# ruivieira/ccfd-demo-summit

Hardware: AMD Instinct MI355X
Metric: transactions/sec (whole node) + p50 scoring latency at 1/2/4/8 MI355X (higher is better)
Workload: dtype bf16

## Files before the change

ccfd_demo_summit_amd/engine/stream_engine.py:

```python
from __future__ import annotations

import ctypes as C
import threading
import time
from dataclasses import dataclass, field
from typing import Dict, List, Optional

import numpy as np
import torch

from ..ops._lib import (BATCH_TRACE_DTYPE, BIN_FORMATS, ENGINE_FLAG_FULL, FLAGGED_DTYPE, SCORED_DTYPE, MODEL_IDS,
                        N_COUNTER_SLOTS, ROW_FORMATS, EngineConfig, EngineStats, Flagged, check, last_error, lib)
from ..ops._lib import (CNT_SHADOW_ABSDIFF_E6, CNT_SHADOW_BOTH, CNT_SHADOW_FRAUD, CNT_SHADOW_PROBA_E6,
                        CNT_SHADOW_ROWS)
from ..ops.kernels import ROW_BYTES, DeviceModel, check_shadow_pair

N_FEATURES = 30
WIRE_ROW_F32 = 16
G32_ROW_F32 = 8
G20_ROW_F32 = 5
INPUT_MODES = {"dma": 0, "zerocopy": 1}
OUTPUT_MODES = {"zerocopy": 0, "dma": 1}


# ... 615 lines not shown
        out = np.zeros(getattr(self, "_trace_cap", 0), BATCH_TRACE_DTYPE)
        if out.size == 0:
            return out
        n = lib().ccfd_engine_trace_read(C.c_void_p(self.h), out.ctypes.data, out.size)
        if n < 0:
            raise RuntimeError(f"ccfd_engine_trace_read failed: {last_error()}")
        return out[:n]

    def progress(self) -> Dict[str, int]:
        v = np.zeros(5, np.int64)
        if getattr(self, "h", None):
            lib().ccfd_engine_progress(C.c_void_p(self.h), v.ctypes.data)
        return {"submitted": int(v[0]), "completed": int(v[1]), "persist_posted": int(v[2]),
                "persist_resident": int(v[3]), "in_flight": int(v[4])}

    def emergency_stop(self, timeout_ms: int = 5000) -> int:
        if not getattr(self, "h", None):
            return 0
        return int(lib().ccfd_engine_emergency_stop(C.c_void_p(self.h), int(timeout_ms)))

    def cursor(self, partition: int) -> int:
        return int(lib().ccfd_engine_cursor(C.c_void_p(self.h), int(partition)))
```

ccfd_demo_summit_amd/ops/_lib.py:

```python
from __future__ import annotations

import ctypes as C
import os
import threading
from pathlib import Path

import torch

_NATIVE = Path(__file__).resolve().parents[1] / "_native"
_SAN = os.environ.get("CCFD_SANITIZE", "")
LIB_PATH = _NATIVE / (f"libccfd_hip_{_SAN.replace(',', '_')}.so" if _SAN else "libccfd_hip.so")
if os.environ.get("CCFD_LIB_PATH"):
    LIB_PATH = Path(os.environ["CCFD_LIB_PATH"]).resolve()

MODEL_LR, MODEL_MLP, MODEL_GBDT, MODEL_FOREST = 0, 1, 2, 3
MODEL_IDS = {"lr": MODEL_LR, "mlp": MODEL_MLP, "gbdt": MODEL_GBDT, "forest": MODEL_FOREST}
N_COUNTER_SLOTS = 64
ENGINE_FLAG_FULL = 1
CNT_WIRE_STALE = 4
CNT_SHADOW_ROWS, CNT_SHADOW_FRAUD, CNT_SHADOW_BOTH, CNT_SHADOW_PROBA_E6, CNT_SHADOW_ABSDIFF_E6 = 40, 41, 42, 43, 44
ARG_WIRE_W64, ARG_WIRE_G32, ARG_WIRE_G20 = 2, 4, 8
ROW_FORMATS = {"f32": 0, "w64": 1, "g32": 2, "g20": 3}
BIN_FORMATS = ("g32", "g20")

# ... 115 lines not shown
        L.ccfd_engine_drain_scored.argtypes = [C.c_void_p, C.c_void_p, C.c_int64]
        L.ccfd_engine_drain_scored.restype = C.c_int64
        L.ccfd_engine_scored_dropped.argtypes = [C.c_void_p]
        L.ccfd_engine_scored_dropped.restype = C.c_int64
        L.ccfd_engine_serve_start.argtypes = [C.c_void_p, C.c_int64, C.c_int64]
        L.ccfd_engine_serve_stop.argtypes = [C.c_void_p]
        L.ccfd_engine_serve_hold.argtypes = [C.c_void_p, C.c_int]
        L.ccfd_engine_serve_stats.argtypes = [C.c_void_p, C.POINTER(EngineStats), C.POINTER(C.c_int64)]
        L.ccfd_engine_serve_collect.argtypes = [C.c_void_p, C.POINTER(EngineStats), C.c_void_p, C.c_int64,
                                                C.POINTER(C.c_int64), C.c_void_p, C.c_int64, C.POINTER(C.c_int64)]
        L.ccfd_engine_cursor.argtypes = [C.c_void_p, C.c_int]
        L.ccfd_engine_cursor.restype = C.c_int64
        L.ccfd_engine_reset_stats.argtypes = [C.c_void_p]
        L.ccfd_engine_progress.argtypes = [C.c_void_p, C.c_void_p]
        L.ccfd_engine_emergency_stop.argtypes = [C.c_void_p, C.c_int]
        L.ccfd_engine_trace_enable.argtypes = [C.c_void_p, C.c_int32]
        L.ccfd_engine_trace_read.argtypes = [C.c_void_p, C.c_void_p, C.c_int32]
        L.ccfd_engine_set_ring.argtypes = [C.c_void_p, C.c_int, C.c_void_p, C.c_void_p, C.c_void_p, C.c_int64]
        L.ccfd_engine_ring_acquire.argtypes = [C.c_void_p, C.c_int, C.c_int64, C.POINTER(C.c_int64)]
        L.ccfd_engine_ring_acquire.restype = C.c_int64
        L.ccfd_engine_ring_commit.argtypes = [C.c_void_p, C.c_int, C.c_int64]
        L.ccfd_engine_ring_commit_at.argtypes = [C.c_void_p, C.c_int, C.c_int64, C.c_int64]
        L.ccfd_engine_run.argtypes = [C.c_void_p, C.c_int64, C.c_int64, C.POINTER(EngineStats)]
        L.ccfd_crc32c.argtypes = [C.c_char_p, C.c_size_t, C.c_uint32]
        L.ccfd_crc32c.restype = C.c_uint32
        L.ccfd_parse_json_batch.argtypes = [C.c_void_p, C.c_void_p, C.c_int64, C.c_void_p, C.c_void_p,
                                            C.c_void_p]
        L.ccfd_parse_json_batch.restype = C.c_int64
        L.ccfd_parse_json_batch_w64.argtypes = [C.c_void_p, C.c_void_p, C.c_int64, C.c_void_p, C.c_void_p,
                                                C.c_void_p]
# ... 33 lines not shown
```

csrc/engine/engine.cpp:

```cpp
#include <hip/hip_runtime_api.h>

#include <algorithm>
#include <atomic>
#include <chrono>
#include <cmath>
#include <cstdio>
#include <cstdlib>
#include <cstring>
#include <deque>
#include <memory>
#include <mutex>
#include <string>
#include <thread>
#include <utility>
#include <vector>

#include <sys/prctl.h>

#if defined(__x86_64__)
#include <immintrin.h>
#endif

#include "../include/ccfd_abi.h"
#include "spsc_ring.h"

namespace ccfd {
void set_error(const std::string& e);
#ifdef CCFD_EXP_ITEM_TRACE
int item_trace_dump(const char* path);
#endif
}

namespace {

using ccfd::set_error;

constexpr int kMaxDevices = 64;
std::atomic<int> g_persist_engines[kMaxDevices];

inline int64_t now_ns() {
  return std::chrono::duration_cast<std::chrono::nanoseconds>(
             std::chrono::steady_clock::now().time_since_epoch()).count();
}

#define HIPCHK(expr)                                                          \
  do {                                                                        \
    hipError_t _e = (expr);                                                   \
    if (_e != hipSuccess) {                                                   \
      set_error(std::string(#expr ": ") + hipGetErrorString(_e));             \
      return -4;                                                              \
    }                                                                         \
  } while (0)

// ... 227 lines not shown
    return 0;
  }

  bool persistent = false;
  bool persist_counted = false;
  bool coherent_out = true;
  uint64_t launches = 0;
  int rowf = CCFD_N_FEATURES;
  int amount_f = CCFD_N_FEATURES - 1;
  int wire_flag = 0;
  bool debug_sync = false;
  float* sync_stage = nullptr;
  const float* sync_stage_dev = nullptr;
  int sync_zc_rows = 512;
  int64_t idle_flush_ns = 20'000;
  ccfd_persist_ctl* pctl = nullptr;
  ccfd_persist_desc* pdesc = nullptr;
  ccfd_persist_dev* pdev = nullptr;
  hipStream_t pstream = nullptr;
  bool prunning = false;
  int persist_C = 0;
  int persist_tpw = 1;
  bool persist_pipe = false;
  const void* shadow_blob = nullptr;
  int64_t completed_upto = 0;
  std::vector<int64_t> flip_seq;

  int persist_init() {
    const bool g32 = cfg.model == CCFD_MODEL_GBDT && cfg.wire >= 2;
    if (cfg.model != CCFD_MODEL_MLP && cfg.model != CCFD_MODEL_LR && !g32) {
      set_error(cfg.model == CCFD_MODEL_FOREST
                    ? "persistent exec_mode has no general-tree (forest) kernel: use exec_mode launch"
                    : "persistent exec_mode supports the MLP and LR models, and GBDT on G32 / G20 rows");
      return -1;
    }
    if (cfg.output_mode != 0 || cfg.depth > CCFD_PERSIST_MAX_RING) {
      set_error("persistent exec_mode needs zero-copy outputs and depth <= 64");
      return -1;
    }
    if (cfg.device < 0 || cfg.device >= kMaxDevices) { set_error("device index out of range"); return -1; }
    {
      int max_q = 4;
      if (const char* e = std::getenv("GPU_MAX_HW_QUEUES")) max_q = std::max(1, std::atoi(e));
      if (g_persist_engines[cfg.device].fetch_add(1) >= max_q) {
        g_persist_engines[cfg.device].fetch_sub(1);
        set_error("more persistent engines on one device than GPU_MAX_HW_QUEUES in one process: their "
                  "kernels would share a hardware queue");
        return -1;
      }
      persist_counted = true;
    }
    void* p = nullptr;
    HIPCHK(hipHostMalloc(&p, sizeof(ccfd_persist_ctl), hipHostMallocMapped | hipHostMallocPortable | hipHostMallocCoherent));
    std::memset(p, 0, sizeof(ccfd_persist_ctl));
    pctl = static_cast<ccfd_persist_ctl*>(p);
    HIPCHK(hipHostMalloc(&p, sizeof(ccfd_persist_desc) * cfg.depth,
                         hipHostMallocMapped | hipHostMallocPortable | hipHostMallocCoherent));
    std::memset(p, 0, sizeof(ccfd_persist_desc) * cfg.depth);
    pdesc = static_cast<ccfd_persist_desc*>(p);
    const bool w64 = (wire_flag & CCFD_ARG_WIRE_W64) != 0;
    const bool big_trees = g32 && cfg.gbdt_trees * cfg.gbdt_depth > 1200;
    int item_rows = big_trees ? 256 : (g32 || (w64 && cfg.model == CCFD_MODEL_MLP)) ? 512 : CCFD_PERSIST_ITEM_ROWS;
    if (const char* e = std::getenv("CCFD_PERSIST_ITEM_ROWS")) {
      const int v = std::atoi(e);
      if (v == 256 || v == 512 || v == 1024 || (!g32 && (v == 64 || v == 128))) item_rows = v;
    }
    persist_tpw = g32 ? item_rows / 256 : item_rows / 64;
    persist_pipe = false;
    const bool g32_pipe_ok = g32 && !big_trees && ((long)cfg.gbdt_trees << cfg.gbdt_depth) <= 16384;
    if ((w64 && cfg.model == CCFD_MODEL_MLP) || g32_pipe_ok) {
      if (cfg.persist_items == 2) persist_pipe = true;
      else if (cfg.persist_items == 0)
        if (const char* e = std::getenv("CCFD_PERSIST_PIPE")) persist_pipe = std::atoi(e) != 0;
    }
    if (persist_pipe && g32) {
      item_rows = 512;
      persist_tpw = 2;
    } else if (persist_pipe) {
      item_rows = 128;
      if (const char* e = std::getenv("CCFD_PERSIST_ITEM_ROWS")) if (std::atoi(e) == 64) item_rows = 64;
      persist_tpw = item_rows / 64;
    }
    const int C = (cfg.max_batch + item_rows - 1) / item_rows;
    ccfd_persist_dev init{};
    for (int i = 0; i < CCFD_PERSIST_MAX_RING; ++i) init.remaining[i] = (unsigned)C;
    HIPCHK(hipMalloc(reinterpret_cast<void**>(&pdev), sizeof(ccfd_persist_dev)));
    HIPCHK(hipMemcpy(pdev, &init, sizeof(init), hipMemcpyHostToDevice));
    {
      int least = 0, greatest = 0;
      HIPCHK(hipDeviceGetStreamPriorityRange(&least, &greatest));
      HIPCHK(hipStreamCreateWithPriority(&pstream, hipStreamNonBlocking, least));
    }
    persist_C = C;
    persistent = true;
    return 0;
  }

  int persist_launch() {
    ccfd_persist_dev init{};
    init.work_next = (unsigned long long)pctl->posted * (unsigned long long)persist_C;
    init.posted = pctl->posted;
    init.stop = 0;
    for (int i = 0; i < CCFD_PERSIST_MAX_RING; ++i) init.remaining[i] = (unsigned)persist_C;
    HIPCHK(hipMemcpyAsync(pdev, &init, sizeof(init), hipMemcpyHostToDevice, pstream));
    HIPCHK(hipStreamSynchronize(pstream));
    __atomic_store_n(&pctl->stop, 0ull, __ATOMIC_RELEASE);
    ccfd_persist_args a{};
    void* d = nullptr;
    HIPCHK(hipHostGetDevicePointer(&d, pctl, 0));
    a.ctl = static_cast<ccfd_persist_ctl*>(d);
    HIPCHK(hipHostGetDevicePointer(&d, pdesc, 0));
    a.desc = static_cast<const ccfd_persist_desc*>(d);
    a.dev = pdev;
    a.ring = cfg.depth;
    a.items_per_batch = persist_C;
    a.tiles_per_wave = persist_tpw;
    a.flags = (coherent_out ? CCFD_ARG_FENCE_COHERENT : CCFD_ARG_FENCE_SYS) | wire_flag |
              (persist_pipe ? CCFD_ARG_PIPE_ITEMS : 0);
    a.model = cfg.model;
    a.threshold = cfg.threshold;
    a.rules = cfg.rules;
    a.blob = cfg.blob;
    a.counters[0] = cfg.counters[0];
    a.counters[1] = cfg.counters[1];
    a.gbdt_trees = cfg.gbdt_trees;
    a.gbdt_depth = cfg.gbdt_depth;
    const bool big_trees = (wire_flag & CCFD_ARG_WIRE_G32) && cfg.gbdt_trees * cfg.gbdt_depth > 1200;
    const int grid = cfg.persist_grid > 0 ? cfg.persist_grid
                     : persist_pipe ? CCFD_PERSIST_GRID
                     : (wire_flag & CCFD_ARG_WIRE_W64) ? CCFD_PERSIST_GRID_W64
                     : big_trees ? 4 * CCFD_PERSIST_GRID
                     : (wire_flag & CCFD_ARG_WIRE_G20) ? CCFD_PERSIST_GRID_G20 : CCFD_PERSIST_GRID;
    int rc;
    if (shadow_blob) {
      ccfd_persist_shadow_args sa{};
      sa.base = a;
      sa.shadow_blob = shadow_blob;
      rc = ccfd_persist_launch_shadow(&sa, grid, pstream);
    } else {
      rc = ccfd_persist_launch(&a, grid, pstream);
    }
    if (rc) { set_error("persistent kernel launch failed"); return rc; }
    prunning = true;
    return 0;
  }

  int persist_halt() {
    if (!prunning) return 0;
    __atomic_store_n(&pctl->stop, 1ull, __ATOMIC_RELEASE);
    const int64_t t0 = now_ns();
    hipError_t q;
    while ((q = hipStreamQuery(pstream)) == hipErrorNotReady) {
      if (now_ns() - t0 > 20ll * 1000000000ll) { set_error("persistent kernel did not stop"); return -6; }
      std::this_thread::sleep_for(std::chrono::microseconds(20));
    }
    prunning = false;
    if (q != hipSuccess) { set_error(std::string("persistent kernel: ") + hipGetErrorString(q)); return -4; }
    return 0;
  }

  void persist_free() {
    if (!persistent) {
      if (pstream) (void)hipStreamDestroy(pstream);
      if (pdev) (void)hipFree(pdev);
      if (pdesc) (void)hipHostFree(pdesc);
      if (pctl) (void)hipHostFree(pctl);
      pstream = nullptr; pdev = nullptr; pdesc = nullptr; pctl = nullptr;
      if (persist_counted) g_persist_engines[cfg.device].fetch_sub(1);
      persist_counted = false;
      return;
    }
    for (auto& s : slots) {
      if (s.busy) wait_done(s);
      if (s.use_flag) { s.busy = false; s.use_flag = false; s.done_ptr = nullptr; }
    }
    persist_halt();
#ifdef CCFD_EXP_ITEM_TRACE
    if (const char* out = std::getenv("CCFD_ITEM_TRACE_OUT")) {
      static int k = 0;
      const std::string path = std::string(out) + "." + std::to_string(k++);
      ccfd::item_trace_dump(path.c_str());
    }
#endif
    (void)hipStreamDestroy(pstream);
    (void)hipFree(pdev);
    (void)hipHostFree(pdesc);
    (void)hipHostFree(pctl);
    if (persist_counted) g_persist_engines[cfg.device].fetch_sub(1);
    persist_counted = false;
    persistent = false;
  }

  void persist_post(Slot& s, const float* x_dev) {
    const uint64_t sq = seq;
    ccfd_persist_desc& d = pdesc[sq % cfg.depth];
    d.x = x_dev;
    d.proba = s.h_proba_dev;
    d.route = s.h_route_dev;
    d.flag_idx = s.h_flag_dev;
    d.n = s.rows;
    d.epoch = epoch & 1;
    d.seq = sq;
    s.expect = sq + 1;
    s.use_flag = true;
    s.done_ptr = reinterpret_cast<volatile unsigned long long*>(pctl->done[sq % cfg.depth]);
    arm(s);
    __atomic_store_n(&pctl->posted, sq + 1, __ATOMIC_RELEASE);
  }

  ~Engine() {
    stamper_stop.store(true);
    if (stamper.joinable()) stamper.join();
    if (std::getenv("CCFD_STAMPER_DEBUG"))
      std::fprintf(stderr, "[engine] completion stamps used %llu missed %llu rejected %llu written %llu iters %llu\n",
                   (unsigned long long)stamp_used, (unsigned long long)stamp_missed,
                   (unsigned long long)stamp_rejected, (unsigned long long)stamps_written.load(),
                   (unsigned long long)stamper_iters.load());
    (void)hipSetDevice(cfg.device);
    persist_free();
    if (sync_stage) (void)hipHostFree(sync_stage);
    for (auto& s : slots) {
      if (s.busy) wait_done(s);
// ... 238 lines not shown
  }

  int submit(Slot& s, const float* x_dev_or_host, const float* x_host, int rows, hipStream_t stream,
             bool force_dma = false, bool force_zc = false) {
    s.t_submit = now_ns();
    s.seq_no = (int64_t)seq;
    struct Acc { uint64_t& a; int64_t t0; ~Acc() { a += now_ns() - t0; } } acc{t_submit_ns, s.t_submit};
    const float* xk = x_dev_or_host;
    if (persistent) {
      if ((cfg.input_mode == 0 || force_dma) && !force_zc) {
        HIPCHK(hipMemcpy(s.d_x, x_host, (size_t)rows * rowf * sizeof(float), hipMemcpyHostToDevice));
        xk = s.d_x;
      }
      if (!prunning) { int rc = persist_launch(); if (rc) return rc; }
      s.rows = rows;
      persist_post(s, xk);
      s.busy = true;
      return 0;
    }
    if ((cfg.input_mode == 0 || force_dma) && !force_zc) {
      HIPCHK(hipMemcpyAsync(s.d_x, x_host, (size_t)rows * rowf * sizeof(float),
                            hipMemcpyHostToDevice, stream));
      xk = s.d_x;
    }
    ccfd_score_args a{};
    a.x = xk; a.ld = rowf; a.n = rows; a.model = cfg.model; a.blob = cfg.blob;
    a.threshold = cfg.threshold; a.gbdt_trees = cfg.gbdt_trees; a.gbdt_depth = cfg.gbdt_depth;
    a.rules = cfg.rules;
    a.proba = cfg.output_mode == 1 ? s.d_proba : s.h_proba_dev;
    a.route = cfg.output_mode == 1 ? s.d_route : s.h_route_dev;
    a.counters = cfg.counters[epoch & 1];
// ... 221 lines not shown
      static const char* const kKind[] = {"lr", "mlp", "gbdt", "forest"};
      if (cfg.model != CCFD_MODEL_MLP) {
        set_error(std::string("shadow model refused: the engine's champion is ") +
                  (cfg.model >= 0 && cfg.model < 4 ? kKind[cfg.model] : "unknown") +
                  "; only an MLP champion on W64 rows can carry a shadow");
        return -1;
      }
      if (cfg.wire != 1) {
        set_error("shadow model refused: the engine scores an MLP on f32 rows; shadow scoring needs W64 rows");
        return -1;
      }
      if (cfg.rules != nullptr) {
        set_error("shadow model refused: the engine routes by a rule program; shadow scoring routes by threshold only");
        return -1;
      }
      if (persistent && persist_pipe) {
        set_error("shadow model refused: pipelined persistent items (persist_items = 2 / CCFD_PERSIST_PIPE) "
                  "have no shadow kernel; use claimed items");
        return -1;
      }
      if (persistent && persist_tpw != 2 && persist_tpw != 4 && persist_tpw != 8) {
        set_error("shadow model refused: persistent items of " + std::to_string(64 * persist_tpw) +
                  " rows; the shadow kernel takes items of 128, 256 or 512 rows");
        return -1;
      }
    }
    HIPCHK(hipSetDevice(cfg.device));
    int rc = drain_all();
    if (rc) return rc;
    if (persistent && prunning) { rc = persist_halt(); if (rc) return rc; }
    shadow_blob = blob;
    return 0;
  }

  int flip_epoch(void* side_stream) {
    HIPCHK(hipSetDevice(cfg.device));
    const int closed = epoch & 1;
// ... 341 lines not shown
  return (int64_t)e->s_dropped;
}

int64_t ccfd_engine_cursor(void* eng, int partition) {
  auto* e = static_cast<Engine*>(eng);
  if (partition < 0 || partition >= (int)e->parts.size()) return -1;
  Partition& P = *e->parts[partition];
  return P.ring ? P.rr.released_count() : P.cursor;
}

int ccfd_engine_progress(void* eng, int64_t* out) {
  auto* e = static_cast<Engine*>(eng);
  if (!out) return -1;
  out[0] = (int64_t)e->seq;
  out[1] = e->completed_upto;
  out[2] = e->persistent && e->pctl ? (int64_t)__atomic_load_n(&e->pctl->posted, __ATOMIC_RELAXED) : -1;
  out[3] = e->prunning ? 1 : 0;
  int64_t busy = 0;
  for (const auto& s : e->slots) busy += s.busy ? 1 : 0;
  out[4] = busy;
  return 0;
}

int ccfd_engine_emergency_stop(void* eng, int timeout_ms) {
  auto* e = static_cast<Engine*>(eng);
  if (!e->persistent || !e->pctl || !e->prunning) return 0;
  __atomic_store_n(&e->pctl->stop, 1ull, __ATOMIC_RELEASE);
  const int64_t t0 = now_ns();
  while (hipStreamQuery(e->pstream) == hipErrorNotReady) {
    if (now_ns() - t0 > (int64_t)timeout_ms * 1000000ll) return -6;
    std::this_thread::sleep_for(std::chrono::microseconds(200));
  }
  return 0;
}

int ccfd_engine_set_amount(void* eng, int partition, const float* amount) {
  auto* e = static_cast<Engine*>(eng);
  ApiLock lk(e);
  if (partition < 0 || partition >= (int)e->parts.size()) { set_error("bad partition index"); return -1; }
  int rc = e->drain_all();
  if (rc) return rc;
  e->parts[partition]->amount = amount;
  return 0;
}

int ccfd_engine_set_ring(void* eng, int partition, float* feats, uint64_t* ids, uint32_t* customer,
                         int64_t capacity) {
  ApiLock lk(static_cast<Engine*>(eng));
  return static_cast<Engine*>(eng)->set_ring(partition, feats, ids, customer, capacity);
// ... 35 lines not shown
  const uint64_t cap = e->trace.size();
  if (cap == 0) return 0;
  const uint64_t have = std::min<uint64_t>(e->trace_n, cap);
  const uint64_t n = std::min<uint64_t>(have, (uint64_t)max);
  const uint64_t first = e->trace_n - n;
  for (uint64_t i = 0; i < n; ++i) out[i] = e->trace[(first + i) % cap];
  return (int)n;
}

void ccfd_engine_reset_stats(void* eng) {
  auto* e = static_cast<Engine*>(eng);
  ApiLock lk(e);
  e->reset_latency();
  e->t_submit_ns = e->t_wait_ns = e->t_complete_ns = 0;
  e->dev_batches = e->dev_exec_ns = 0;
  std::memset(e->dev_hist, 0, sizeof(e->dev_hist));
  std::memset(e->dev_hist_rows, 0, sizeof(e->dev_hist_rows));
}

}
```

csrc/include/ccfd_abi.h:

```cpp
#pragma once
#include <stddef.h>
#include <stdint.h>

#ifdef __cplusplus
extern "C" {
#endif

enum ccfd_model_kind { CCFD_MODEL_LR = 0, CCFD_MODEL_MLP = 1, CCFD_MODEL_GBDT = 2, CCFD_MODEL_FOREST = 3 };

enum ccfd_counter_slot {
  CCFD_CNT_INCOMING = 0,
  CCFD_CNT_FRAUD = 1,
  CCFD_CNT_STANDARD = 2,
  CCFD_CNT_PROBA_E6 = 3,
  CCFD_CNT_WIRE_STALE = 4,
  CCFD_CNT_HIST_STD = 8,
  CCFD_CNT_HIST_FRAUD = 24,
  CCFD_CNT_SHADOW_ROWS = 40,
  CCFD_CNT_SHADOW_FRAUD = 41,
  CCFD_CNT_SHADOW_BOTH = 42,
  CCFD_CNT_SHADOW_PROBA_E6 = 43,
  CCFD_CNT_SHADOW_ABSDIFF_E6 = 44,
  CCFD_CNT_SLOTS = 64
};
// ... 125 lines not shown
  const ccfd_persist_desc* desc;
  ccfd_persist_dev* dev;
  int32_t ring;
  int32_t items_per_batch;
  int32_t model;
  float threshold;
  int32_t tiles_per_wave;
  int32_t flags;
  const void* blob;
  unsigned long long* counters[2];
  const ccfd_rule_prog* rules;
  int32_t gbdt_trees, gbdt_depth;
} ccfd_persist_args;

int ccfd_persist_launch(const ccfd_persist_args* a, int grid, void* stream);

typedef struct ccfd_persist_shadow_args {
  ccfd_persist_args base;
  const void* shadow_blob;
} ccfd_persist_shadow_args;
int ccfd_persist_launch_shadow(const ccfd_persist_shadow_args* a, int grid, void* stream);

void* ccfd_host_alloc(size_t bytes);
int ccfd_host_free(void* p);
void* ccfd_host_device_ptr(void* host_ptr);

typedef struct ccfd_engine_config {
  int32_t device;
  int32_t model;
  const void* blob;
// ... 68 lines not shown
int ccfd_engine_set_log(void* eng, int partition, const float* feats, const uint64_t* ids,
                        const uint32_t* customer, int64_t n_rows, int64_t cursor);
int ccfd_engine_pump(void* eng, int64_t n_batches, int32_t batch_rows, int32_t drain,
                     ccfd_engine_stats* st);
int ccfd_engine_score_sync(void* eng, const float* x, int32_t n, float* proba_out, uint8_t* route_out);
int ccfd_engine_flip_epoch(void* eng, void* side_stream);
int ccfd_engine_epoch_complete(void* eng, int64_t flip_count);
int ccfd_engine_set_blob(void* eng, const void* blob);
int ccfd_engine_set_shadow(void* eng, const void* blob);
int64_t ccfd_engine_drain_flagged(void* eng, ccfd_flagged* out, int64_t max);
int64_t ccfd_engine_cursor(void* eng, int partition);
int ccfd_engine_scored_enable(void* eng, int64_t capacity);
int64_t ccfd_engine_drain_scored(void* eng, ccfd_scored* out, int64_t max);
int64_t ccfd_engine_scored_dropped(void* eng);
int ccfd_engine_progress(void* eng, int64_t* out5);
int ccfd_engine_emergency_stop(void* eng, int timeout_ms);
int ccfd_engine_set_amount(void* eng, int partition, const float* amount);

int ccfd_engine_set_ring(void* eng, int partition, float* feats, uint64_t* ids, uint32_t* customer,
                         int64_t capacity);
int64_t ccfd_engine_ring_acquire(void* eng, int partition, int64_t want, int64_t* row);
int ccfd_engine_ring_commit(void* eng, int partition, int64_t n);
int ccfd_engine_ring_commit_at(void* eng, int partition, int64_t n, int64_t origin_ns);
int ccfd_engine_run(void* eng, int64_t budget_us, int64_t flush_us, ccfd_engine_stats* st);
void ccfd_engine_reset_stats(void* eng);
int ccfd_engine_serve_start(void* eng, int64_t budget_us, int64_t flush_us);
int ccfd_engine_serve_stop(void* eng);
int ccfd_engine_serve_hold(void* eng, int hold);
int ccfd_engine_serve_stats(void* eng, ccfd_engine_stats* out, int64_t* iters);
int ccfd_engine_serve_collect(void* eng, ccfd_engine_stats* out, ccfd_flagged* flagged, int64_t max_flagged,
// ... 72 lines not shown
```

csrc/kernels/score_persist.hip:

```cpp
#include <type_traits>

#include "mlp_core.h"
#include "persist_core.h"
#include "rules.h"

namespace ccfd {

int launch_persist_gbdt_g32(const ccfd_persist_args& a, int grid, hipStream_t s);

namespace {

template <int kModel, bool kR>
__global__ __launch_bounds__(256) void persist_kernel(ccfd_persist_args a) {
  __shared__ __attribute__((aligned(16))) char sblob[kMlpBlobWire];
  __shared__ __attribute__((aligned(16))) float sx[4][kTileRows * kF + 4];
  __shared__ EpilogueLds epi;
  __shared__ ccfd_persist_desc sdesc;
  __shared__ unsigned long long s_item;
  __shared__ int s_cmd;

  const int tid = threadIdx.x;
  const int lane = tid & 63, wave = tid >> 6;
  const int g = lane >> 4, c = lane & 15;
  const int C = a.items_per_batch;

  if (kModel == CCFD_MODEL_MLP)
    mlp_stage(a.blob, sblob, tid, 256, (a.flags & CCFD_ARG_WIRE_W64) ? kMlpBlobWire : kMlpBlob);
  else for (int i = tid; i < 448 / 16; i += 256) reinterpret_cast<int4*>(sblob)[i] = reinterpret_cast<const int4*>(a.blob)[i];
  epi_init(epi);
  __syncthreads();

  MlpLane L{};
  MlpWireLane LW{};
  float wm[8];
  if (kModel == CCFD_MODEL_MLP) {
    L = mlp_lane(sblob, g);
    LW = mlp_wire_lane(sblob);
  } else {
    const unsigned flags = *reinterpret_cast<const unsigned*>(sblob + 4);
    L.b3 = *reinterpret_cast<const float*>(sblob + 8);
    L.log_amount = (flags & 1u) != 0;
    const float* mu = reinterpret_cast<const float*>(sblob + 64) + 8 * g;
    const float* isg = reinterpret_cast<const float*>(sblob + 192) + 8 * g;
    const float* w = reinterpret_cast<const float*>(sblob + 320) + 8 * g;
#pragma unroll
    for (int j = 0; j < 8; ++j) { L.mu[j] = mu[j]; L.isg[j] = isg[j]; wm[j] = w[j]; }
  }
  float* tile_lds = sx[wave];
  unsigned long long posted_cache = 0;

  if (blockIdx.x == 0) {
    if (wave == 0) persist_doorbell(a, lane);
    return;
  }

  for (;;) {
    if (tid == 0) persist_claim(a, C, posted_cache, sdesc, s_item, s_cmd);
    __syncthreads();
    if (s_cmd) break;

    const unsigned long long item = s_item;
    const ccfd_persist_desc dsc = sdesc;
    const int chunk = (int)(item % (unsigned long long)C);
    const int slot = (int)(dsc.seq % (unsigned long long)a.ring);
    const int n = dsc.n;
    const float* x = dsc.x;
    const int kTilesPerWave = a.tiles_per_wave;
    const int tile0 = chunk * (4 * kTilesPerWave) + wave;
    if (chunk == 0 && tid == 0)
      __hip_atomic_store(&a.dev->tstart[slot], wall_clock64(), __ATOMIC_RELAXED, __HIP_MEMORY_SCOPE_AGENT);
    auto avail = [&](int t) { return min(kTileRows, n - t * kTileRows) * kF * 4; };
    const bool wire = (a.flags & CCFD_ARG_WIRE_W64) != 0;
    const unsigned char* xw = reinterpret_cast<const unsigned char*>(x);
    unsigned nf_w = 0, nv_w = 0;
    unsigned long long ps_w = 0;
    auto lr_p = [&](float (&xv)[8]) __attribute__((always_inline)) {
      if (g == 3) { xv[6] = 0.f; xv[7] = 0.f; if (L.log_amount) xv[5] = log1pf(fmaxf(xv[5], 0.f)); }
      float z = 0.f;
#pragma unroll
      for (int j = 0; j < 8; ++j) z = fmaf((xv[j] - L.mu[j]) * L.isg[j], wm[j], z);
      z += __shfl_xor(z, 16);
      z += __shfl_xor(z, 32);
      return sigmoid(z + L.b3);
    };
    auto finish = [&](float p, float amount, int tile, float (&xr)[8]) __attribute__((always_inline)) {
      const int row = tile * kTileRows + c;
      const bool valid = row < n;
// ... 94 lines not shown
          p = lr_p(xv);
        }
        finish(p, amount, tile, xr);
      }
    }
    ps_w = wave_sum_u64(ps_w);
    if (lane == 0 && nv_w) {
      atomicAdd(&epi.fraud, nf_w);
      atomicAdd(&epi.rows, nv_w);
      atomicAdd(&epi.psum_e6, ps_w);
    }
    persist_item_done(a, epi, dsc, slot, C, tid);
  }
}

template <bool kR, int T>
__global__ __launch_bounds__(256) void persist_pipe_kernel(ccfd_persist_args a) {
  static_assert(T == 1 || T == 2, "64- or 128-row items");
  __shared__ __attribute__((aligned(16))) char sblob[kMlpBlobWire];
  __shared__ EpilogueLds epi;
  __shared__ ccfd_persist_desc sdesc[2];
  __shared__ int s_pre, s_cmd;

  const int tid = threadIdx.x;
  const int lane = tid & 63, wave = tid >> 6;
  const int g = lane >> 4, c = lane & 15;
  const int C = a.items_per_batch;
  mlp_stage(a.blob, sblob, tid, 256, kMlpBlobWire);
  epi_init(epi);
  __syncthreads();
  if (blockIdx.x == 0) {
    if (wave == 0) persist_doorbell(a, lane);
    return;
  }
  const MlpWireLane LW = mlp_wire_lane(sblob);
  const unsigned long long W = gridDim.x - 1;
  unsigned long long item = __hip_atomic_load(&a.dev->work_next, __ATOMIC_RELAXED, __HIP_MEMORY_SCOPE_AGENT) +
                            (unsigned long long)(blockIdx.x - 1);
  unsigned long long posted_cache = 0;

  auto stamp = [&](const ccfd_persist_desc& d, unsigned long long it) __attribute__((always_inline)) {
    if (it % (unsigned long long)C == 0)
      __hip_atomic_store(&a.dev->tstart[d.seq % (unsigned long long)a.ring], wall_clock64(), __ATOMIC_RELAXED,
                         __HIP_MEMORY_SCOPE_AGENT);
  };
  auto issue = [&](const ccfd_persist_desc& d, unsigned long long it, WireRegs (&r)[T]) __attribute__((always_inline)) {
    const int tile0 = (int)(it % (unsigned long long)C) * (4 * T) + wave;
    const unsigned char* xw = reinterpret_cast<const unsigned char*>(d.x);
#pragma unroll
    for (int k = 0; k < T; ++k) wire_issue(xw, d.n, tile0 + 4 * k, c, g, r[k]);
  };
  auto score = [&](const ccfd_persist_desc& d, unsigned long long it, const WireRegs (&r_in)[T]) __attribute__((always_inline)) {
    const int slot = (int)(d.seq % (unsigned long long)a.ring);
// ... 72 lines not shown
    s_cmd = persist_wait_far(a, C, posted_cache, item, sdesc[0]);
    if (!s_cmd) stamp(sdesc[0], item);
  }
  __syncthreads();
  if (s_cmd) return;
  WireRegs ra[T], rb[T];
  issue(sdesc[0], item, ra);
  for (;;) {
    if (stage(sdesc[0], ra, sdesc[1], rb, item)) break;
    item += W;
    if (stage(sdesc[1], rb, sdesc[0], ra, item)) break;
    item += W;
  }
}

}

}

extern "C" int ccfd_persist_launch(const ccfd_persist_args* a, int grid, void* stream) {
  using namespace ccfd;
  if (!a || !a->ctl || !a->desc || !a->dev || !a->blob) return -1;
  if (a->ring <= 0 || a->ring > CCFD_PERSIST_MAX_RING || a->items_per_batch <= 0 || a->tiles_per_wave <= 0) return -2;
  hipStream_t s = reinterpret_cast<hipStream_t>(stream);
  if (a->model == CCFD_MODEL_MLP && (a->flags & CCFD_ARG_PIPE_ITEMS)) {
    if (!(a->flags & CCFD_ARG_WIRE_W64) || grid < 2) return -2;
    const bool r = a->rules != nullptr;
    switch (a->tiles_per_wave) {
      case 1: if (r) hipLaunchKernelGGL((persist_pipe_kernel<true, 1>), dim3(grid), dim3(256), 0, s, *a);
              else hipLaunchKernelGGL((persist_pipe_kernel<false, 1>), dim3(grid), dim3(256), 0, s, *a); break;
      case 2: if (r) hipLaunchKernelGGL((persist_pipe_kernel<true, 2>), dim3(grid), dim3(256), 0, s, *a);
              else hipLaunchKernelGGL((persist_pipe_kernel<false, 2>), dim3(grid), dim3(256), 0, s, *a); break;
      default: return -2;
    }
  } else if (a->model == CCFD_MODEL_MLP) {
    if (a->rules) hipLaunchKernelGGL((persist_kernel<CCFD_MODEL_MLP, true>), dim3(grid), dim3(256), 0, s, *a);
    else hipLaunchKernelGGL((persist_kernel<CCFD_MODEL_MLP, false>), dim3(grid), dim3(256), 0, s, *a);
  } else if (a->model == CCFD_MODEL_LR) {
    if (a->rules) hipLaunchKernelGGL((persist_kernel<CCFD_MODEL_LR, true>), dim3(grid), dim3(256), 0, s, *a);
    else hipLaunchKernelGGL((persist_kernel<CCFD_MODEL_LR, false>), dim3(grid), dim3(256), 0, s, *a);
  } else if (a->model == CCFD_MODEL_GBDT && (a->flags & CCFD_ARG_WIRE_G32)) {
    return launch_persist_gbdt_g32(*a, grid, s);
  } else {
    return -3;
  }
  return hipGetLastError() == hipSuccess ? 0 : -5;
}
```

Baseline: 891.3 million.

## Split persistent MLP kernel into claimed and pipelined lanes routed by load

Adds a dual-lane persistent kernel: one launch hosts a claimed-items lane with large items and a pipelined lane with 128-row items. Each lane has its own control, descriptor and device state. The host sends a batch to the low-latency pipelined lane when fewer than K slots are busy, and to the claimed lane under load. The aim is to cut p50 latency at light load while keeping throughput under heavy load. The cost is that the persistent grid's blocks are split between two lanes, and the change adds host bookkeeping and complexity to launch, halt and stop.

```diff
diff --git a/ccfd_demo_summit_amd/engine/stream_engine.py b/ccfd_demo_summit_amd/engine/stream_engine.py
--- a/ccfd_demo_summit_amd/engine/stream_engine.py
+++ b/ccfd_demo_summit_amd/engine/stream_engine.py
@@ -653,6 +653,12 @@
         return {"submitted": int(v[0]), "completed": int(v[1]), "persist_posted": int(v[2]),
                 "persist_resident": int(v[3]), "in_flight": int(v[4])}
 
+    def lane_counts(self) -> Dict[str, int]:
+        v = np.zeros(2, np.int64)
+        if getattr(self, "h", None):
+            lib().ccfd_engine_lane_counts(C.c_void_p(self.h), v.ctypes.data)
+        return {"claimed": int(v[0]), "pipelined": int(v[1])}
+
     def emergency_stop(self, timeout_ms: int = 5000) -> int:
         if not getattr(self, "h", None):
             return 0
diff --git a/ccfd_demo_summit_amd/ops/_lib.py b/ccfd_demo_summit_amd/ops/_lib.py
--- a/ccfd_demo_summit_amd/ops/_lib.py
+++ b/ccfd_demo_summit_amd/ops/_lib.py
@@ -153,6 +153,9 @@
         L.ccfd_engine_reset_stats.argtypes = [C.c_void_p]
         L.ccfd_engine_progress.argtypes = [C.c_void_p, C.c_void_p]
         L.ccfd_engine_emergency_stop.argtypes = [C.c_void_p, C.c_int]
+        if hasattr(L, "ccfd_engine_lane_counts"):
+            L.ccfd_engine_lane_counts.argtypes = [C.c_void_p, C.c_void_p]
+            L.ccfd_engine_route_lane.argtypes = [C.c_int, C.c_int]
         L.ccfd_engine_trace_enable.argtypes = [C.c_void_p, C.c_int32]
         L.ccfd_engine_trace_read.argtypes = [C.c_void_p, C.c_void_p, C.c_int32]
         L.ccfd_engine_set_ring.argtypes = [C.c_void_p, C.c_int, C.c_void_p, C.c_void_p, C.c_void_p, C.c_int64]
diff --git a/csrc/engine/engine.cpp b/csrc/engine/engine.cpp
--- a/csrc/engine/engine.cpp
+++ b/csrc/engine/engine.cpp
@@ -37,6 +37,8 @@
 
 constexpr int kMaxDevices = 64;
 std::atomic<int> g_persist_engines[kMaxDevices];
+
+constexpr int kDefaultLaneK = 4;
 
 inline int64_t now_ns() {
   return std::chrono::duration_cast<std::chrono::nanoseconds>(
@@ -294,14 +296,22 @@
   const float* sync_stage_dev = nullptr;
   int sync_zc_rows = 512;
   int64_t idle_flush_ns = 20'000;
-  ccfd_persist_ctl* pctl = nullptr;
-  ccfd_persist_desc* pdesc = nullptr;
-  ccfd_persist_dev* pdev = nullptr;
+  struct PersistLane {
+    ccfd_persist_ctl* ctl = nullptr;
+    ccfd_persist_desc* desc = nullptr;
+    ccfd_persist_dev* dev = nullptr;
+    int C = 0;
+    int tpw = 1;
+    bool pipe = false;
+    uint64_t posted = 0;
+    uint64_t posted_stat = 0;
+  };
+  PersistLane lanes[2];
+  bool dual = false;
+  int lane_k = 0;
+  int lane_grid = 0;
   hipStream_t pstream = nullptr;
   bool prunning = false;
-  int persist_C = 0;
-  int persist_tpw = 1;
-  bool persist_pipe = false;
   const void* shadow_blob = nullptr;
   int64_t completed_upto = 0;
   std::vector<int64_t> flip_seq;
@@ -330,14 +340,6 @@
       }
       persist_counted = true;
     }
-    void* p = nullptr;
-    HIPCHK(hipHostMalloc(&p, sizeof(ccfd_persist_ctl), hipHostMallocMapped | hipHostMallocPortable | hipHostMallocCoherent));
-    std::memset(p, 0, sizeof(ccfd_persist_ctl));
-    pctl = static_cast<ccfd_persist_ctl*>(p);
-    HIPCHK(hipHostMalloc(&p, sizeof(ccfd_persist_desc) * cfg.depth,
-                         hipHostMallocMapped | hipHostMallocPortable | hipHostMallocCoherent));
-    std::memset(p, 0, sizeof(ccfd_persist_desc) * cfg.depth);
-    pdesc = static_cast<ccfd_persist_desc*>(p);
     const bool w64 = (wire_flag & CCFD_ARG_WIRE_W64) != 0;
     const bool big_trees = g32 && cfg.gbdt_trees * cfg.gbdt_depth > 1200;
     int item_rows = big_trees ? 256 : (g32 || (w64 && cfg.model == CCFD_MODEL_MLP)) ? 512 : CCFD_PERSIST_ITEM_ROWS;
@@ -345,8 +347,8 @@
       const int v = std::atoi(e);
       if (v == 256 || v == 512 || v == 1024 || (!g32 && (v == 64 || v == 128))) item_rows = v;
     }
-    persist_tpw = g32 ? item_rows / 256 : item_rows / 64;
-    persist_pipe = false;
+    int persist_tpw = g32 ? item_rows / 256 : item_rows / 64;
+    bool persist_pipe = false;
     const bool g32_pipe_ok = g32 && !big_trees && ((long)cfg.gbdt_trees << cfg.gbdt_depth) <= 16384;
     if ((w64 && cfg.model == CCFD_MODEL_MLP) || g32_pipe_ok) {
       if (cfg.persist_items == 2) persist_pipe = true;
@@ -361,42 +363,76 @@
       if (const char* e = std::getenv("CCFD_PERSIST_ITEM_ROWS")) if (std::atoi(e) == 64) item_rows = 64;
       persist_tpw = item_rows / 64;
     }
-    const int C = (cfg.max_batch + item_rows - 1) / item_rows;
-    ccfd_persist_dev init{};
-    for (int i = 0; i < CCFD_PERSIST_MAX_RING; ++i) init.remaining[i] = (unsigned)C;
-    HIPCHK(hipMalloc(reinterpret_cast<void**>(&pdev), sizeof(ccfd_persist_dev)));
-    HIPCHK(hipMemcpy(pdev, &init, sizeof(init), hipMemcpyHostToDevice));
+    lane_k = kDefaultLaneK;
+    const char* e_k = std::getenv("CCFD_PERSIST_LANE_K");
+    if (e_k) lane_k = std::max(0, std::atoi(e_k));
+    if (const char* e = std::getenv("CCFD_PERSIST_LANE_GRID")) lane_grid = std::max(0, std::atoi(e));
+    const bool sized = cfg.persist_grid > 0 || std::getenv("CCFD_PERSIST_ITEM_ROWS") != nullptr;
+    dual = w64 && cfg.model == CCFD_MODEL_MLP && cfg.persist_items == 0 && !std::getenv("CCFD_PERSIST_PIPE") &&
+           lane_k > 0 && (!sized || e_k != nullptr);
+    if (dual && lane_grid == 1) { set_error("CCFD_PERSIST_LANE_GRID: a lane needs its doorbell and a worker (>= 2)"); return -1; }
+    {
+      int rc = lane_alloc(lanes[0], item_rows, persist_tpw, persist_pipe);
+      if (!rc && dual) rc = lane_alloc(lanes[1], 128, 2, true);
+      if (rc) return rc;
+    }
     {
       int least = 0, greatest = 0;
       HIPCHK(hipDeviceGetStreamPriorityRange(&least, &greatest));
       HIPCHK(hipStreamCreateWithPriority(&pstream, hipStreamNonBlocking, least));
     }
-    persist_C = C;
     persistent = true;
     return 0;
   }
 
-  int persist_launch() {
+  int lane_alloc(PersistLane& L, int item_rows, int tpw, bool pipe) {
+    void* p = nullptr;
+    HIPCHK(hipHostMalloc(&p, sizeof(ccfd_persist_ctl), hipHostMallocMapped | hipHostMallocPortable | hipHostMallocCoherent));
+    std::memset(p, 0, sizeof(ccfd_persist_ctl));
+    L.ctl = static_cast<ccfd_persist_ctl*>(p);
+    HIPCHK(hipHostMalloc(&p, sizeof(ccfd_persist_desc) * cfg.depth,
+                         hipHostMallocMapped | hipHostMallocPortable | hipHostMallocCoherent));
+    std::memset(p, 0, sizeof(ccfd_persist_desc) * cfg.depth);
+    L.desc = static_cast<ccfd_persist_desc*>(p);
+    L.C = (cfg.max_batch + item_rows - 1) / item_rows;
+    L.tpw = tpw;
+    L.pipe = pipe;
     ccfd_persist_dev init{};
-    init.work_next = (unsigned long long)pctl->posted * (unsigned long long)persist_C;
-    init.posted = pctl->posted;
+    for (int i = 0; i < CCFD_PERSIST_MAX_RING; ++i) init.remaining[i] = (unsigned)L.C;
+    HIPCHK(hipMalloc(reinterpret_cast<void**>(&L.dev), sizeof(ccfd_persist_dev)));
+    HIPCHK(hipMemcpy(L.dev, &init, sizeof(init), hipMemcpyHostToDevice));
+    return 0;
+  }
+
+  void lane_free(PersistLane& L) {
+    if (L.dev) (void)hipFree(L.dev);
+    if (L.desc) (void)hipHostFree(L.desc);
+    if (L.ctl) (void)hipHostFree(L.ctl);
+    L.dev = nullptr; L.desc = nullptr; L.ctl = nullptr;
+  }
+
+  bool dual_active() const { return dual && shadow_blob == nullptr; }
+
+  int lane_args(PersistLane& L, ccfd_persist_args& a) {
+    ccfd_persist_dev init{};
+    init.work_next = (unsigned long long)L.posted * (unsigned long long)L.C;
+    init.posted = L.posted;
     init.stop = 0;
-    for (int i = 0; i < CCFD_PERSIST_MAX_RING; ++i) init.remaining[i] = (unsigned)persist_C;
-    HIPCHK(hipMemcpyAsync(pdev, &init, sizeof(init), hipMemcpyHostToDevice, pstream));
+    for (int i = 0; i < CCFD_PERSIST_MAX_RING; ++i) init.remaining[i] = (unsigned)L.C;
+    HIPCHK(hipMemcpyAsync(L.dev, &init, sizeof(init), hipMemcpyHostToDevice, pstream));
     HIPCHK(hipStreamSynchronize(pstream));
-    __atomic_store_n(&pctl->stop, 0ull, __ATOMIC_RELEASE);
-    ccfd_persist_args a{};
+    __atomic_store_n(&L.ctl->stop, 0ull, __ATOMIC_RELEASE);
     void* d = nullptr;
-    HIPCHK(hipHostGetDevicePointer(&d, pctl, 0));
+    HIPCHK(hipHostGetDevicePointer(&d, L.ctl, 0));
     a.ctl = static_cast<ccfd_persist_ctl*>(d);
-    HIPCHK(hipHostGetDevicePointer(&d, pdesc, 0));
+    HIPCHK(hipHostGetDevicePointer(&d, L.desc, 0));
     a.desc = static_cast<const ccfd_persist_desc*>(d);
-    a.dev = pdev;
+    a.dev = L.dev;
     a.ring = cfg.depth;
-    a.items_per_batch = persist_C;
-    a.tiles_per_wave = persist_tpw;
+    a.items_per_batch = L.C;
+    a.tiles_per_wave = L.tpw;
     a.flags = (coherent_out ? CCFD_ARG_FENCE_COHERENT : CCFD_ARG_FENCE_SYS) | wire_flag |
-              (persist_pipe ? CCFD_ARG_PIPE_ITEMS : 0);
+              (L.pipe ? CCFD_ARG_PIPE_ITEMS : 0);
     a.model = cfg.model;
     a.threshold = cfg.threshold;
     a.rules = cfg.rules;
@@ -405,9 +441,16 @@
     a.counters[1] = cfg.counters[1];
     a.gbdt_trees = cfg.gbdt_trees;
     a.gbdt_depth = cfg.gbdt_depth;
+    return 0;
+  }
+
+  int persist_launch() {
+    ccfd_persist_args a{}, ap{};
+    { int rc = lane_args(lanes[0], a); if (rc) return rc; }
+    if (dual_active()) { int rc = lane_args(lanes[1], ap); if (rc) return rc; }
     const bool big_trees = (wire_flag & CCFD_ARG_WIRE_G32) && cfg.gbdt_trees * cfg.gbdt_depth > 1200;
     const int grid = cfg.persist_grid > 0 ? cfg.persist_grid
-                     : persist_pipe ? CCFD_PERSIST_GRID
+                     : lanes[0].pipe ? CCFD_PERSIST_GRID
                      : (wire_flag & CCFD_ARG_WIRE_W64) ? CCFD_PERSIST_GRID_W64
                      : big_trees ? 4 * CCFD_PERSIST_GRID
                      : (wire_flag & CCFD_ARG_WIRE_G20) ? CCFD_PERSIST_GRID_G20 : CCFD_PERSIST_GRID;
@@ -417,6 +460,8 @@
       sa.base = a;
       sa.shadow_blob = shadow_blob;
       rc = ccfd_persist_launch_shadow(&sa, grid, pstream);
+    } else if (dual_active()) {
+      rc = ccfd_persist_launch_dual(&a, grid, &ap, lane_grid > 0 ? lane_grid : CCFD_PERSIST_GRID, pstream);
     } else {
       rc = ccfd_persist_launch(&a, grid, pstream);
     }
@@ -425,9 +470,14 @@
     return 0;
   }
 
+  void persist_stop_all() {
+    for (auto& L : lanes)
+      if (L.ctl) __atomic_store_n(&L.ctl->stop, 1ull, __ATOMIC_RELEASE);
+  }
+
   int persist_halt() {
     if (!prunning) return 0;
-    __atomic_store_n(&pctl->stop, 1ull, __ATOMIC_RELEASE);
+    persist_stop_all();
     const int64_t t0 = now_ns();
     hipError_t q;
     while ((q = hipStreamQuery(pstream)) == hipErrorNotReady) {
@@ -442,10 +492,8 @@
   void persist_free() {
     if (!persistent) {
       if (pstream) (void)hipStreamDestroy(pstream);
-      if (pdev) (void)hipFree(pdev);
-      if (pdesc) (void)hipHostFree(pdesc);
-      if (pctl) (void)hipHostFree(pctl);
-      pstream = nullptr; pdev = nullptr; pdesc = nullptr; pctl = nullptr;
+      for (auto& L : lanes) lane_free(L);
+      pstream = nullptr;
       if (persist_counted) g_persist_engines[cfg.device].fetch_sub(1);
       persist_counted = false;
       return;
@@ -463,17 +511,25 @@
     }
 #endif
     (void)hipStreamDestroy(pstream);
-    (void)hipFree(pdev);
-    (void)hipHostFree(pdesc);
-    (void)hipHostFree(pctl);
+    for (auto& L : lanes) lane_free(L);
     if (persist_counted) g_persist_engines[cfg.device].fetch_sub(1);
     persist_counted = false;
     persistent = false;
   }
 
-  void persist_post(Slot& s, const float* x_dev) {
-    const uint64_t sq = seq;
-    ccfd_persist_desc& d = pdesc[sq % cfg.depth];
+  static int route_lane(int busy, int k) { return busy < k ? 1 : 0; }
+
+  int pick_lane() const {
+    if (!dual_active()) return 0;
+    int busy = 0;
+    for (const auto& s : slots) busy += s.busy ? 1 : 0;
+    return route_lane(busy, lane_k);
+  }
+
+  void persist_post(Slot& s, const float* x_dev, int li) {
+    PersistLane& L = lanes[li];
+    const uint64_t sq = L.posted;
+    ccfd_persist_desc& d = L.desc[sq % cfg.depth];
     d.x = x_dev;
     d.proba = s.h_proba_dev;
     d.route = s.h_route_dev;
@@ -483,9 +539,11 @@
     d.seq = sq;
     s.expect = sq + 1;
     s.use_flag = true;
-    s.done_ptr = reinterpret_cast<volatile unsigned long long*>(pctl->done[sq % cfg.depth]);
+    s.done_ptr = reinterpret_cast<volatile unsigned long long*>(L.ctl->done[sq % cfg.depth]);
     arm(s);
-    __atomic_store_n(&pctl->posted, sq + 1, __ATOMIC_RELEASE);
+    L.posted = sq + 1;
+    ++L.posted_stat;
+    __atomic_store_n(&L.ctl->posted, sq + 1, __ATOMIC_RELEASE);
   }
 
   ~Engine() {
@@ -754,7 +812,7 @@
       }
       if (!prunning) { int rc = persist_launch(); if (rc) return rc; }
       s.rows = rows;
-      persist_post(s, xk);
+      persist_post(s, xk, pick_lane());
       s.busy = true;
       return 0;
     }
@@ -1006,13 +1064,13 @@
         set_error("shadow model refused: the engine routes by a rule program; shadow scoring routes by threshold only");
         return -1;
       }
-      if (persistent && persist_pipe) {
+      if (persistent && lanes[0].pipe) {
         set_error("shadow model refused: pipelined persistent items (persist_items = 2 / CCFD_PERSIST_PIPE) "
                   "have no shadow kernel; use claimed items");
         return -1;
       }
-      if (persistent && persist_tpw != 2 && persist_tpw != 4 && persist_tpw != 8) {
-        set_error("shadow model refused: persistent items of " + std::to_string(64 * persist_tpw) +
+      if (persistent && lanes[0].tpw != 2 && lanes[0].tpw != 4 && lanes[0].tpw != 8) {
+        set_error("shadow model refused: persistent items of " + std::to_string(64 * lanes[0].tpw) +
                   " rows; the shadow kernel takes items of 128, 256 or 512 rows");
         return -1;
       }
@@ -1384,7 +1442,12 @@
   if (!out) return -1;
   out[0] = (int64_t)e->seq;
   out[1] = e->completed_upto;
-  out[2] = e->persistent && e->pctl ? (int64_t)__atomic_load_n(&e->pctl->posted, __ATOMIC_RELAXED) : -1;
+  out[2] = -1;
+  if (e->persistent && e->lanes[0].ctl) {
+    out[2] = 0;
+    for (const auto& L : e->lanes)
+      if (L.ctl) out[2] += (int64_t)__atomic_load_n(&L.ctl->posted, __ATOMIC_RELAXED);
+  }
   out[3] = e->prunning ? 1 : 0;
   int64_t busy = 0;
   for (const auto& s : e->slots) busy += s.busy ? 1 : 0;
@@ -1394,8 +1457,8 @@
 
 int ccfd_engine_emergency_stop(void* eng, int timeout_ms) {
   auto* e = static_cast<Engine*>(eng);
-  if (!e->persistent || !e->pctl || !e->prunning) return 0;
-  __atomic_store_n(&e->pctl->stop, 1ull, __ATOMIC_RELEASE);
+  if (!e->persistent || !e->lanes[0].ctl || !e->prunning) return 0;
+  e->persist_stop_all();
   const int64_t t0 = now_ns();
   while (hipStreamQuery(e->pstream) == hipErrorNotReady) {
     if (now_ns() - t0 > (int64_t)timeout_ms * 1000000ll) return -6;
@@ -1403,6 +1466,18 @@
   }
   return 0;
 }
+
+int ccfd_engine_lane_counts(void* eng, int64_t* out) {
+  auto* e = static_cast<Engine*>(eng);
+  if (!out) return -1;
+  out[0] = out[1] = 0;
+  if (!e->persistent) return 0;
+  for (const auto& L : e->lanes)
+    if (L.ctl) out[L.pipe ? 1 : 0] += (int64_t)L.posted_stat;
+  return 0;
+}
+
+int ccfd_engine_route_lane(int busy_slots, int lane_k) { return Engine::route_lane(busy_slots, lane_k); }
 
 int ccfd_engine_set_amount(void* eng, int partition, const float* amount) {
   auto* e = static_cast<Engine*>(eng);
@@ -1468,6 +1543,7 @@
   e->reset_latency();
   e->t_submit_ns = e->t_wait_ns = e->t_complete_ns = 0;
   e->dev_batches = e->dev_exec_ns = 0;
+  for (auto& L : e->lanes) L.posted_stat = 0;
   std::memset(e->dev_hist, 0, sizeof(e->dev_hist));
   std::memset(e->dev_hist_rows, 0, sizeof(e->dev_hist_rows));
 }
diff --git a/csrc/include/ccfd_abi.h b/csrc/include/ccfd_abi.h
--- a/csrc/include/ccfd_abi.h
+++ b/csrc/include/ccfd_abi.h
@@ -163,6 +163,8 @@
 } ccfd_persist_args;
 
 int ccfd_persist_launch(const ccfd_persist_args* a, int grid, void* stream);
+int ccfd_persist_launch_dual(const ccfd_persist_args* claimed, int grid_claimed, const ccfd_persist_args* piped,
+                             int grid_piped, void* stream);
 
 typedef struct ccfd_persist_shadow_args {
   ccfd_persist_args base;
@@ -261,6 +263,8 @@
 int64_t ccfd_engine_drain_scored(void* eng, ccfd_scored* out, int64_t max);
 int64_t ccfd_engine_scored_dropped(void* eng);
 int ccfd_engine_progress(void* eng, int64_t* out5);
+int ccfd_engine_lane_counts(void* eng, int64_t* out2);
+int ccfd_engine_route_lane(int busy_slots, int lane_k);
 int ccfd_engine_emergency_stop(void* eng, int timeout_ms);
 int ccfd_engine_set_amount(void* eng, int partition, const float* amount);
 
diff --git a/csrc/kernels/score_persist.hip b/csrc/kernels/score_persist.hip
--- a/csrc/kernels/score_persist.hip
+++ b/csrc/kernels/score_persist.hip
@@ -10,22 +10,19 @@
 
 namespace {
 
-template <int kModel, bool kR>
-__global__ __launch_bounds__(256) void persist_kernel(ccfd_persist_args a) {
-  __shared__ __attribute__((aligned(16))) char sblob[kMlpBlobWire];
-  __shared__ __attribute__((aligned(16))) float sx[4][kTileRows * kF + 4];
-  __shared__ EpilogueLds epi;
-  __shared__ ccfd_persist_desc sdesc;
-  __shared__ unsigned long long s_item;
-  __shared__ int s_cmd;
-
+constexpr int kSxWave = kTileRows * kF + 4;
+
+template <int kModel, bool kR, bool kWireOnly>
+__device__ __forceinline__ void persist_claimed_body(const ccfd_persist_args& a, const int block, char* sblob,
+                                                     float* sx, EpilogueLds& epi, ccfd_persist_desc& sdesc,
+                                                     unsigned long long& s_item, int& s_cmd) {
   const int tid = threadIdx.x;
   const int lane = tid & 63, wave = tid >> 6;
   const int g = lane >> 4, c = lane & 15;
   const int C = a.items_per_batch;
 
   if (kModel == CCFD_MODEL_MLP)
-    mlp_stage(a.blob, sblob, tid, 256, (a.flags & CCFD_ARG_WIRE_W64) ? kMlpBlobWire : kMlpBlob);
+    mlp_stage(a.blob, sblob, tid, 256, (kWireOnly || (a.flags & CCFD_ARG_WIRE_W64)) ? kMlpBlobWire : kMlpBlob);
   else for (int i = tid; i < 448 / 16; i += 256) reinterpret_cast<int4*>(sblob)[i] = reinterpret_cast<const int4*>(a.blob)[i];
   epi_init(epi);
   __syncthreads();
@@ -46,10 +43,10 @@
 #pragma unroll
     for (int j = 0; j < 8; ++j) { L.mu[j] = mu[j]; L.isg[j] = isg[j]; wm[j] = w[j]; }
   }
-  float* tile_lds = sx[wave];
+  float* tile_lds = kWireOnly ? nullptr : sx + wave * kSxWave;
   unsigned long long posted_cache = 0;
 
-  if (blockIdx.x == 0) {
+  if (block == 0) {
     if (wave == 0) persist_doorbell(a, lane);
     return;
   }
@@ -70,7 +67,7 @@
     if (chunk == 0 && tid == 0)
       __hip_atomic_store(&a.dev->tstart[slot], wall_clock64(), __ATOMIC_RELAXED, __HIP_MEMORY_SCOPE_AGENT);
     auto avail = [&](int t) { return min(kTileRows, n - t * kTileRows) * kF * 4; };
-    const bool wire = (a.flags & CCFD_ARG_WIRE_W64) != 0;
+    const bool wire = kWireOnly || (a.flags & CCFD_ARG_WIRE_W64) != 0;
     const unsigned char* xw = reinterpret_cast<const unsigned char*>(x);
     unsigned nf_w = 0, nv_w = 0;
     unsigned long long ps_w = 0;
@@ -195,14 +192,22 @@
   }
 }
 
+template <int kModel, bool kR>
+__global__ __launch_bounds__(256) void persist_kernel(ccfd_persist_args a) {
+  __shared__ __attribute__((aligned(16))) char sblob[kMlpBlobWire];
+  __shared__ __attribute__((aligned(16))) float sx[4][kSxWave];
+  __shared__ EpilogueLds epi;
+  __shared__ ccfd_persist_desc sdesc;
+  __shared__ unsigned long long s_item;
+  __shared__ int s_cmd;
+  persist_claimed_body<kModel, kR, false>(a, (int)blockIdx.x, sblob, &sx[0][0], epi, sdesc, s_item, s_cmd);
+}
+
 template <bool kR, int T>
-__global__ __launch_bounds__(256) void persist_pipe_kernel(ccfd_persist_args a) {
+__device__ __forceinline__ void persist_pipe_body(const ccfd_persist_args& a, const int block, const int nblocks,
+                                                  char* sblob, EpilogueLds& epi, ccfd_persist_desc (&sdesc)[2],
+                                                  int& s_pre, int& s_cmd) {
   static_assert(T == 1 || T == 2, "64- or 128-row items");
-  __shared__ __attribute__((aligned(16))) char sblob[kMlpBlobWire];
-  __shared__ EpilogueLds epi;
-  __shared__ ccfd_persist_desc sdesc[2];
-  __shared__ int s_pre, s_cmd;
-
   const int tid = threadIdx.x;
   const int lane = tid & 63, wave = tid >> 6;
   const int g = lane >> 4, c = lane & 15;
@@ -210,14 +215,14 @@
   mlp_stage(a.blob, sblob, tid, 256, kMlpBlobWire);
   epi_init(epi);
   __syncthreads();
-  if (blockIdx.x == 0) {
+  if (block == 0) {
     if (wave == 0) persist_doorbell(a, lane);
     return;
   }
   const MlpWireLane LW = mlp_wire_lane(sblob);
-  const unsigned long long W = gridDim.x - 1;
+  const unsigned long long W = (unsigned long long)(nblocks - 1);
   unsigned long long item = __hip_atomic_load(&a.dev->work_next, __ATOMIC_RELAXED, __HIP_MEMORY_SCOPE_AGENT) +
-                            (unsigned long long)(blockIdx.x - 1);
+                            (unsigned long long)(block - 1);
   unsigned long long posted_cache = 0;
 
   auto stamp = [&](const ccfd_persist_desc& d, unsigned long long it) __attribute__((always_inline)) {
@@ -320,14 +325,46 @@
   }
 }
 
-}
-
+template <bool kR, int T>
+__global__ __launch_bounds__(256) void persist_pipe_kernel(ccfd_persist_args a) {
+  __shared__ __attribute__((aligned(16))) char sblob[kMlpBlobWire];
+  __shared__ EpilogueLds epi;
+  __shared__ ccfd_persist_desc sdesc[2];
+  __shared__ int s_pre, s_cmd;
+  persist_pipe_body<kR, T>(a, (int)blockIdx.x, (int)gridDim.x, sblob, epi, sdesc, s_pre, s_cmd);
+}
+
+template <bool kR, int T>
+__global__ __launch_bounds__(256) void persist_dual_kernel(ccfd_persist_args claimed, ccfd_persist_args piped,
+                                                           int grid_claimed) {
+  __shared__ __attribute__((aligned(16))) char sblob[kMlpBlobWire];
+  __shared__ EpilogueLds epi;
+  __shared__ ccfd_persist_desc sdesc[2];
+  __shared__ unsigned long long s_item;
+  __shared__ int s_pre, s_cmd;
+  const int block = (int)blockIdx.x;
+  if (block < grid_claimed)
+    persist_claimed_body<CCFD_MODEL_MLP, kR, true>(claimed, block, sblob, nullptr, epi, sdesc[0], s_item, s_cmd);
+  else
+    persist_pipe_body<kR, T>(piped, block - grid_claimed, (int)gridDim.x - grid_claimed, sblob, epi, sdesc, s_pre,
+                             s_cmd);
+}
+
+}
+
+}
+
+namespace {
+int persist_args_check(const ccfd_persist_args* a) {
+  if (!a || !a->ctl || !a->desc || !a->dev || !a->blob) return -1;
+  if (a->ring <= 0 || a->ring > CCFD_PERSIST_MAX_RING || a->items_per_batch <= 0 || a->tiles_per_wave <= 0) return -2;
+  return 0;
+}
 }
 
 extern "C" int ccfd_persist_launch(const ccfd_persist_args* a, int grid, void* stream) {
   using namespace ccfd;
-  if (!a || !a->ctl || !a->desc || !a->dev || !a->blob) return -1;
-  if (a->ring <= 0 || a->ring > CCFD_PERSIST_MAX_RING || a->items_per_batch <= 0 || a->tiles_per_wave <= 0) return -2;
+  if (int rc = persist_args_check(a)) return rc;
   hipStream_t s = reinterpret_cast<hipStream_t>(stream);
   if (a->model == CCFD_MODEL_MLP && (a->flags & CCFD_ARG_PIPE_ITEMS)) {
     if (!(a->flags & CCFD_ARG_WIRE_W64) || grid < 2) return -2;
@@ -352,3 +389,27 @@
   }
   return hipGetLastError() == hipSuccess ? 0 : -5;
 }
+
+extern "C" int ccfd_persist_launch_dual(const ccfd_persist_args* claimed, int grid_claimed,
+                                        const ccfd_persist_args* piped, int grid_piped, void* stream) {
+  using namespace ccfd;
+  if (int rc = persist_args_check(claimed)) return rc;
+  if (int rc = persist_args_check(piped)) return rc;
+  if (claimed->model != CCFD_MODEL_MLP || piped->model != CCFD_MODEL_MLP) return -3;
+  if (!(claimed->flags & CCFD_ARG_WIRE_W64) || !(piped->flags & CCFD_ARG_WIRE_W64)) return -2;
+  if ((claimed->flags & CCFD_ARG_PIPE_ITEMS) || !(piped->flags & CCFD_ARG_PIPE_ITEMS)) return -2;
+  if (grid_claimed < 2 || grid_piped < 2) return -2;
+  if (claimed->ctl == piped->ctl || claimed->desc == piped->desc || claimed->dev == piped->dev) return -2;
+  if (claimed->blob != piped->blob || claimed->rules != piped->rules) return -2;
+  hipStream_t s = reinterpret_cast<hipStream_t>(stream);
+  const dim3 grid(grid_claimed + grid_piped);
+  const bool r = claimed->rules != nullptr;
+  switch (piped->tiles_per_wave) {
+    case 1: if (r) hipLaunchKernelGGL((persist_dual_kernel<true, 1>), grid, dim3(256), 0, s, *claimed, *piped, grid_claimed);
+            else hipLaunchKernelGGL((persist_dual_kernel<false, 1>), grid, dim3(256), 0, s, *claimed, *piped, grid_claimed); break;
+    case 2: if (r) hipLaunchKernelGGL((persist_dual_kernel<true, 2>), grid, dim3(256), 0, s, *claimed, *piped, grid_claimed);
+            else hipLaunchKernelGGL((persist_dual_kernel<false, 2>), grid, dim3(256), 0, s, *claimed, *piped, grid_claimed); break;
+    default: return -2;
+  }
+  return hipGetLastError() == hipSuccess ? 0 : -5;
+}
```

Measured after the change: 890.5 million. Within noise of the previous version (-0.1%).
